# addtt/ladder-vae-pytorch

Hardware: AMD Instinct MI355X
Metric: training images/sec (ELBO step: fwd+bwd+Adamax) (higher is better)
Workload: dtype f32; 1 GPU; CIFAR10-shaped 15-layer LVAE (BASELINE configs[2]): 32x32x3, zdims 32x15, 4 blocks/layer, 64 filters, gated+skip, DMoL-10, dropout 0.2, free bits 1.0; batch_per_gpu=256, global_batch=256, parallelism=dp1, hip_graph=True

## Files before the change

### include/lvae_hip.h

```cpp
#ifndef LVAE_HIP_H
#define LVAE_HIP_H

#include <stddef.h>
#include <stdint.h>

#ifdef __cplusplus
extern "C" {
#endif

#define LVAE_ABI_VERSION 17

#define LVAE_EINVAL (-1)
#define LVAE_EALIGN (-2)
#define LVAE_EWORKSPACE (-3)

enum { LVAE_STATS_BN_FWD = 0, LVAE_STATS_BN_BWD = 1 };
enum { LVAE_PREC_F32 = 0, LVAE_PREC_BF16 = 1 };
enum { LVAE_DT_F32 = 0, LVAE_DT_BF16 = 1 };
enum {
  LVAE_FORM_AUTO = 0,
  LVAE_FORM_F32_MFMA = 1,
  LVAE_FORM_SIX_PRODUCT = 2,
  LVAE_FORM_SIX_PRODUCT_DIRECT = 3
};
// ... 87 lines not shown
  const float* coef;
  const float* dh;
  const float* x;
  const float* add;
  float* dgamma;
  float* dbeta;
  float* out;
  int32_t dh_bf16;
  int32_t reserved_;
  const float* drop;
} lvae_bn_apply;
size_t lvae_conv1x1_gate_bwd_wgrad_workspace(const lvae_conv_desc* d);
int lvae_conv1x1_gate_bwd_wgrad_f32(const lvae_conv_desc* d, const float* dout, const float* ab, const float* y, int32_t act,
                                    float* dw, int64_t dw_sk, int64_t dw_sn, float* db, void* workspace, size_t workspace_bytes,
                                    const lvae_bn_apply* ap, void* stream);

enum { LVAE_RB_PRO_AFFINE = 0, LVAE_RB_PRO_BN_APPLY = 1, LVAE_RB_PRO_GATE_BWD = 2 };
enum { LVAE_RB_EPI_PLAIN = 0, LVAE_RB_EPI_GATE = 1 };
typedef struct lvae_rb_ext {
  int32_t prologue, epilogue;
  const float* gate_w;
  int64_t gate_w_sk, gate_w_sn;
  void* gate_ws;
  int64_t gate_ws_bytes;
  int32_t gate_ws_ready;
  const float* gate_bias;
  int32_t act;
  const float* res;
  float* ab;
  float* out;
// ... 165 lines not shown
```

### ladder-vae-pytorch_amd/_C.py

```python
import ctypes as C
import os

import torch

_HERE = os.path.dirname(os.path.abspath(__file__))
LIB_PATH = os.path.join(_HERE, 'liblvae_hip.so')

ACT = {None: 0, 'none': 0, 'elu': 1, 'relu': 2, 'leakyrelu': 3, 'selu': 4}
GATHER_CONV, GATHER_TRANSPOSED = 0, 1
PREC_F32, PREC_BF16 = 0, 1
DT_F32, DT_BF16 = 0, 1
VARIANT_DIRECT, VARIANT_POS, VARIANT_WINO_F32, VARIANT_WINO_SIX, VARIANT_BF16_DIRECT, VARIANT_SIX_DIRECT = 0, 2, 3, 4, 5, 6
WGRAD_VARIANT_GENERIC, WGRAD_VARIANT_IMG, WGRAD_VARIANT_BF16, WGRAD_VARIANT_WINO, WGRAD_VARIANT_DIRECT_1X1, WGRAD_VARIANT_TILE, WGRAD_VARIANT_THIN = range(7)
FORM_AUTO, FORM_F32_MFMA, FORM_SIX_PRODUCT, FORM_SIX_PRODUCT_DIRECT = 0, 1, 2, 3


class LvaeHipError(RuntimeError):
    pass


class ConvDesc(C.Structure):
    _fields_ = [
        ('x', C.c_void_p), ('x2', C.c_void_p), ('C1', C.c_int32), ('C2', C.c_int32),
        ('w', C.c_void_p), ('w_stap', C.c_int64), ('w_sk', C.c_int64), ('w_sn', C.c_int64),
# ... 47 lines not shown
    'lvae_conv2d_bf16': (C.c_int, [C.POINTER(ConvDesc), _P]),
    'lvae_conv1x1_dgrad_cat_f32': (C.c_int, [C.POINTER(ConvDesc), _P, _I, _P]),
    'lvae_conv2d_stats_rows': (_I, [C.POINTER(ConvDesc)]),
    'lvae_conv2d_variant': (_I, [C.POINTER(ConvDesc)]),
    'lvae_resblock_bf16_storage': (_I, [C.POINTER(ConvDesc)]),
    'lvae_conv2d_folds_bn_finalize': (_I, [C.POINTER(ConvDesc)]),
    'lvae_conv2d_stats_buffer_rows': (_I, [C.POINTER(ConvDesc)]),
    'lvae_conv2d_prepare_entry_bytes': (_Z, []),
    'lvae_conv2d_prepare_entry': (C.c_int, [C.POINTER(ConvDesc), _P]),
    'lvae_conv2d_prepare_weights': (C.c_int, [_P, _I, _I, _P]),
    'lvae_conv1x1_gate_f32': (C.c_int, [C.POINTER(ConvDesc), _P, _I, _P, _P]),
    'lvae_conv1x1_gate_stats_rows': (_I, [C.POINTER(ConvDesc)]),
    'lvae_conv1x1_gate_bwd_f32': (C.c_int, [C.POINTER(ConvDesc), _P, _P, _I, _P, _P]),
    'lvae_conv1x1_gate_bwd_wgrad_workspace': (_Z, [C.POINTER(ConvDesc)]),
    'lvae_conv1x1_gate_bwd_wgrad_f32': (C.c_int, [C.POINTER(ConvDesc), _P, _P, _P, _I, _P, _L, _L, _P, _P, _Z, C.POINTER(BnApply), _P]),
    'lvae_resblock_gate_workspace': (_Z, [C.POINTER(ConvDesc)]),
    'lvae_resblock_gate_prepare_entry': (C.c_int, [C.POINTER(ConvDesc), _P]),
    'lvae_resblock_conv_rows': (_I, [C.POINTER(ConvDesc)]),
    'lvae_resblock_conv_gate_rows': (_I, [C.POINTER(ConvDesc)]),
    'lvae_resblock_conv_workspace': (_Z, [C.POINTER(ConvDesc)]),
    'lvae_resblock_conv_prepare_entry': (C.c_int, [C.POINTER(ConvDesc), _P]),
    'lvae_resblock_conv_f32': (C.c_int, [C.POINTER(ConvDesc), C.POINTER(RbExt), _P]),
    'lvae_conv2d_wgrad_workspace': (_Z, [C.POINTER(ConvDesc)]),
    'lvae_conv2d_wgrad_f32': (C.c_int, [C.POINTER(ConvDesc), _P, _P, _P, _P, _Z, _P]),
    'lvae_conv2d_wgrad_bf16': (C.c_int, [C.POINTER(ConvDesc), _P, _P, _P, _P, _Z, _P]),
    'lvae_conv2d_wgrad_variant': (_I, [C.POINTER(ConvDesc)]),
    'lvae_conv2d_wgrad_apply_ok': (_I, [C.POINTER(ConvDesc)]),
    'lvae_conv2d_wgrad_apply_f32': (C.c_int, [C.POINTER(ConvDesc), C.POINTER(BnApply), _P, _P, _P, _Z, _P]),
    'lvae_conv2d_wgrad_grouped_workspace': (_Z, [C.POINTER(ConvDesc), _I]),
    'lvae_conv2d_wgrad_grouped_f32': (C.c_int, [C.POINTER(ConvDesc), _P, _P, _P, _I, _P, _Z, _P]),
# ... 98 lines not shown
```

### ladder-vae-pytorch_amd/csrc/conv1x1_gate_bwd_fused.hip

```cpp
#include "bf16_frag.h"
#include "lvae_common.h"

namespace lvae {

void wgrad_reduce_launch(const float* slab_w, const float* slab_b, int ksplit, int ntaps, int Cin, int Cout, int64_t stap, int64_t sk,
                         int64_t sn, float* dw, float* db, hipStream_t s);

struct GbfArgs {
  const float* dout;
  const float* ab;
  const float* y;
  const float* w;
  int64_t w_sn;
  const float* drop;
  float* dx;
  float* slab_w;
  float* slab_b;
  int M, ohw, ntiles, act;
  int in_bf16, dx_bf16;
  lvae_bn_apply ap;
};

constexpr int GB_LDA = 132;
constexpr int GB_LDY = 68;

__global__ __launch_bounds__(512) void conv1x1_gate_bwd_fused_kernel(GbfArgs a) {
  kernarg_warmup<(sizeof(GbfArgs) < 1024 ? sizeof(GbfArgs) : 1024)>();
  extern __shared__ __attribute__((aligned(16))) float smem[];
  float* Bs = smem;
  float* As = Bs + 64 * GB_LDA;
  float* Ys = As + 64 * GB_LDA;
  const int t = threadIdx.x, lane = t & 63, wave = t >> 6;
  const bool wg_role = wave >= 4;
  const int wm = (wave & 3) >> 1, wn = wave & 1, li = lane & 31, lh = lane >> 5;
  const f32x4 zero4 = {0.f, 0.f, 0.f, 0.f};
// ... 106 lines not shown
    float* red = As;
    *reinterpret_cast<f32x4*>(red + r0 * 128 + c4) = bs_lo;
    *reinterpret_cast<f32x4*>(red + r0 * 128 + 64 + c4) = bs_hi;
    __syncthreads();
    if (t < 128) {
      float v = 0.f;
#pragma unroll
      for (int g = 0; g < 32; ++g) v += red[g * 128 + t];
      a.slab_b[(size_t)blockIdx.x * 128 + t] = v;
    }
  }
}

constexpr int GBB_LDA = 136;
constexpr int GBB_LDY = 72;
constexpr size_t gbb_lds(int split) {
  return (size_t)split * (64 * GBB_LDA + 64 * GBB_LDY) * 2 + (size_t)64 * GB_LDY * 4 + 6 * 64 * 4 + (split == 3 ? (size_t)8 * 2 * 3 * 64 * 16 : 0);
}

template <int SPLIT, bool S16 = false, bool AP = false, bool ELU = false>
__global__ __launch_bounds__(512) void conv1x1_gate_bwd_fused_bf16_kernel(GbfArgs a) {
  kernarg_warmup<sizeof(GbfArgs)>();
#ifdef LVAE_GBF_DBG
  constexpr int dbg = LVAE_GBF_DBG;
#else
  constexpr int dbg = 0;
#endif
  const int gact = ELU ? LVAE_ACT_ELU : a.act, apact = ELU ? LVAE_ACT_ELU : a.ap.act;
  static_assert(SPLIT == 1 || !S16, "bf16 storage exists for the bf16-operand form only");
  extern __shared__ __attribute__((aligned(16))) unsigned char smem_raw[];
  constexpr int A_PLANE = 64 * GBB_LDA, Y_PLANE = 64 * GBB_LDY;
  __bf16* As = reinterpret_cast<__bf16*>(smem_raw);
  __bf16* Ys = As + SPLIT * A_PLANE;
  float* Os = reinterpret_cast<float*>(Ys + SPLIT * Y_PLANE);
  float* Cf = Os + 64 * GB_LDY;
  const int t = threadIdx.x, lane = t & 63, wave = t >> 6;
  const bool wg_role = wave >= 4;
  const int wm = (wave & 3) >> 1, wn = wave & 1, li = lane & 31, lh = lane >> 5, G = lane >> 4, i16 = lane & 15;
  const f32x4 zero4 = {0.f, 0.f, 0.f, 0.f};

  if (AP) {
    const int q = t & 31, rg = t >> 5, rows = a.ap.rows;
    f32x4 acc = zero4;
    for (int r = rg; r < rows; r += 16 * 8) {
      f32x4 v[8];
#pragma unroll
      for (int u = 0; u < 8; ++u) {
        const int rr = r + 16 * u;
        v[u] = *reinterpret_cast<const f32x4*>(a.ap.parts + (size_t)(rr < rows ? rr : 0) * 128 + q * 4);
      }
// ... 60 lines not shown
  auto prefetch_row = [&](int tile, int u) {
    if (dbg & 1) {
      pg[u] = pa[u] = pb[u] = py[u] = zero4;
      if (AP) px[u] = pd[u] = zero4;
      return;
    }
    const int m = tile * 64 + r0 + 32 * u;
    const size_t mc = m < a.M ? (size_t)m : 0;
    if (AP) {
      pg[u] = load4_dt(a.ap.dh, mc * 64 + c4, ap_dh_bf);
      px[u] = *reinterpret_cast<const f32x4*>(a.ap.x + mc * 64 + c4);
      pd[u] = ap_add ? *reinterpret_cast<const f32x4*>(a.ap.add + mc * 64 + c4) : zero4;
    } else {
      pg[u] = *reinterpret_cast<const f32x4*>(a.dout + mc * 64 + c4);
    }
    pa[u] = load4_dt(a.ab, mc * 128 + c4, a.in_bf16 != 0);
    pb[u] = load4_dt(a.ab, mc * 128 + 64 + c4, a.in_bf16 != 0);
    py[u] = load4_dt(a.y, mc * 64 + c4, a.in_bf16 != 0);
  };
  auto prefetch = [&](int tile) {
    const int m0 = tile * 64;
    if (dbg & 1) {
      pg[0] = pg[1] = zero4;
#pragma unroll
      for (int u = 0; u < IT; ++u) pa[u] = pb[u] = py[u] = zero4;
#pragma unroll
      for (int u = 0; u < (AP ? 2 : 1); ++u) px[u] = pd[u] = zero4;
      qa = qb = qy = bf16x8{0, 0, 0, 0, 0, 0, 0, 0};
      return;
    }
    if (S16) {
      const int m = m0 + r8;
// ... 18 lines not shown
    for (int u = 0; u < IT; ++u) prefetch_row(tile, u);
  };

  f32x16 accw[2];
#pragma unroll
  for (int j = 0; j < 2; ++j)
#pragma unroll
    for (int r = 0; r < 16; ++r) accw[j][r] = 0.f;
  f32x4 bs_lo = zero4, bs_hi = zero4;
  f32x4 bs_lo8 = zero4, bs_hi8 = zero4;
  const int trow = 8 * (G >> 1) + (i16 >> 2), tch = 16 * (G & 1) + 4 * (i16 & 3);
  constexpr int NP = SPLIT == 1 ? 1 : 6;
  constexpr int PA[6] = {SPLIT - 1, 0, SPLIT > 1 ? 1 : 0, SPLIT > 1 ? 1 : 0, 0, 0};
  constexpr int PB[6] = {0, SPLIT - 1, SPLIT > 1 ? 1 : 0, 0, SPLIT > 1 ? 1 : 0, 0};

  int tile = blockIdx.x;
  if (tile < a.ntiles) prefetch(tile);
  for (; tile < a.ntiles; tile += gridDim.x) {
    const int m0 = tile * 64;
    if (S16) {
      f32x4 lo[2] = {zero4, zero4}, hi[2] = {zero4, zero4};
      bf16x8 yv = {0, 0, 0, 0, 0, 0, 0, 0};
      if (m0 + r8 < a.M) {
        if (AP) {
#pragma unroll
          for (int h = 0; h < 2; ++h) {
            pg[h] = ap_value(pg[h], px[h], pd[h], c8 + 4 * h);
            store_wt4(a.ap.out + (size_t)(m0 + r8) * 64 + c8 + 4 * h, pg[h]);
          }
        }
#pragma unroll
        for (int h = 0; h < 2; ++h)
#pragma unroll
          for (int j = 0; j < 4; ++j) {
// ... 9 lines not shown
      bs_hi += hi[0];
      bs_hi8 += hi[1];
      *reinterpret_cast<bf16x8*>(As + r8 * GBB_LDA + c8) = to_bf16x8(lo[0], lo[1]);
      *reinterpret_cast<bf16x8*>(As + r8 * GBB_LDA + 64 + c8) = to_bf16x8(hi[0], hi[1]);
      *reinterpret_cast<bf16x8*>(Ys + r8 * GBB_LDY + c8) = yv;
    } else
#pragma unroll
    for (int u = 0; u < IT; ++u) {
      const int r = r0 + 32 * u;
      f32x4 lo = zero4, hi = zero4, yv = zero4;
      if (m0 + r < a.M) {
        if (AP) {
          pg[u] = ap_value(pg[u], px[u], pd[u], c4);
          if (!(dbg & 4)) store_wt4(a.ap.out + (size_t)(m0 + r) * 64 + c4, pg[u]);
        }
        if (dbg & 8) {
          lo = pg[u] + pa[u];
          hi = pg[u] + pb[u];
        } else
#pragma unroll
        for (int j = 0; j < 4; ++j) {
          const float sg = sigmoidf_(pb[u][j]);
          lo[j] = pg[u][j] * sg * act_grad(pa[u][j], gact);
          hi[j] = pg[u][j] * act_fwd(pa[u][j], gact) * sg * (1.f - sg);
        }
        yv = py[u];
      }
      bs_lo += lo;
      bs_hi += hi;
      if (tile + (int)gridDim.x < a.ntiles) prefetch_row(tile + gridDim.x, u);
      bf16x4 pl[SPLIT], ph[SPLIT], pyv[SPLIT];
      split4<SPLIT>(lo, pl);
      split4<SPLIT>(hi, ph);
      split4<SPLIT>(yv, pyv);
#pragma unroll
      for (int q = 0; q < SPLIT; ++q) {
        *reinterpret_cast<bf16x4*>(As + q * A_PLANE + r * GBB_LDA + c4) = pl[q];
        *reinterpret_cast<bf16x4*>(As + q * A_PLANE + r * GBB_LDA + 64 + c4) = ph[q];
        *reinterpret_cast<bf16x4*>(Ys + q * Y_PLANE + r * GBB_LDY + c4) = pyv[q];
      }
    }
    if (S16 && tile + (int)gridDim.x < a.ntiles) prefetch(tile + gridDim.x);
    lds_barrier();

    if (!wg_role) {
      f32x16 accx;
#pragma unroll
      for (int r = 0; r < 16; ++r) accx[r] = 0.f;
#pragma unroll
      for (int s = 0; s < 8; ++s) {
        bf16x8 af[SPLIT];
#pragma unroll
        for (int q = 0; q < SPLIT; ++q)
          af[q] = *reinterpret_cast<const bf16x8*>(As + q * A_PLANE + (wm * 32 + li) * GBB_LDA + 16 * s + 8 * lh);
// ... 101 lines not shown
  return (int)(ntiles < 256 ? ntiles : 256);
}

size_t conv1x1_gate_bwd_fused_workspace(const lvae_conv_desc* d) {
  static const bool off = tune("LVAE_DISABLE_GATE_FUSED", 0) != 0;
  if (off || d == nullptr) return 0;
  if (d->KH != 1 || d->KW != 1 || d->stride != 1 || d->pad != 0 || d->OH != d->H || d->OW != d->W) return 0;
  if (d->C1 != 128 || d->C2 != 0 || d->Cout != 64 || d->w_sk != 1 || d->w_sn % 4 != 0 || d->in_scale != nullptr) return 0;
  const int64_t M = (int64_t)d->N * d->H * d->W;
  static const int64_t min_m = tune("LVAE_GATE_FUSED_MIN_M", 256 * 64);
  if (M < min_m || M >= ((int64_t)1 << 31)) return 0;
  return (size_t)gbf_nwg(M) * (64 * 128 + 128) * sizeof(float);
}

int conv1x1_gate_bwd_fused(const lvae_conv_desc* d, const float* dout, const float* ab, const float* y, int act, float* dw,
                           int64_t dw_sk, int64_t dw_sn, float* db, void* workspace, const lvae_bn_apply* ap, hipStream_t s) {
  if (!al16f(dout) || !al16f(ab) || !al16f(y) || !al16f(d->w) || !al16f(d->y) || !al16f(d->out_scale) || !al16f(workspace)) return -1000;
  GbfArgs a;
  a.ap = lvae_bn_apply{};
  if (ap != nullptr && ap->parts != nullptr) {
    if (!al16f(ap->parts) || !al16f(ap->coef) || !al16f(ap->dh) || !al16f(ap->x) || !al16f(ap->add) || !al16f(ap->out)) return -1000;
    a.ap = *ap;
  }
  a.dout = dout;
  a.ab = ab;
  a.y = y;
  a.w = d->w;
  a.w_sn = d->w_sn;
  a.drop = d->out_scale;
  a.dx = d->y;
  a.M = d->N * d->H * d->W;
  a.ohw = d->H * d->W;
  a.ntiles = (a.M + 63) / 64;
  a.act = act;
  a.in_bf16 = d->x_dtype == LVAE_DT_BF16;
  a.dx_bf16 = d->y_dtype == LVAE_DT_BF16;
  if ((a.in_bf16 || a.dx_bf16) && d->precision != LVAE_PREC_BF16) return -1000;
  const int nwg = gbf_nwg(a.M);
  a.slab_w = static_cast<float*>(workspace);
  a.slab_b = db ? a.slab_w + (size_t)nwg * 64 * 128 : nullptr;
  constexpr size_t lds = (size_t)(2 * 64 * GB_LDA + 64 * GB_LDY) * sizeof(float);
  static std::atomic<bool> attr_set{false};
  if (!attr_set) {
    hipError_t e = hipFuncSetAttribute(reinterpret_cast<const void*>(conv1x1_gate_bwd_fused_kernel),
                                       hipFuncAttributeMaxDynamicSharedMemorySize, (int)lds);
    if (e != hipSuccess) {
      set_error("conv1x1_gate_bwd_fused: hipFuncSetAttribute failed: %s", hipGetErrorString(e));
      return (int)e;
    }
    attr_set = true;
  }
  const bool f32_mfma = d->form == LVAE_FORM_F32_MFMA;
  const bool with_ap = a.ap.parts != nullptr;
  if (with_ap && (f32_mfma && d->precision != LVAE_PREC_BF16)) {
    set_error("conv1x1_gate_bwd_fused: the deferred BatchNorm-backward apply exists in the bf16-matrix-pipe kernels only (not with LVAE_FORM_F32_MFMA)");
    return LVAE_EINVAL;
  }
  const bool elu = act == LVAE_ACT_ELU && (!with_ap || a.ap.act == LVAE_ACT_ELU);
#define GBF_LAUNCH(SP, S16_, AP_, LDS_)                                                                                                   \
  do {                                                                                                                                    \
    if (elu) hipLaunchKernelGGL((conv1x1_gate_bwd_fused_bf16_kernel<SP, S16_, AP_, true>), dim3(nwg), dim3(512), LDS_, s, a);            \
    else hipLaunchKernelGGL((conv1x1_gate_bwd_fused_bf16_kernel<SP, S16_, AP_, false>), dim3(nwg), dim3(512), LDS_, s, a);               \
  } while (0)
  if (d->precision == LVAE_PREC_BF16) {
    if (with_ap) {
      if (a.in_bf16 && a.dx_bf16) GBF_LAUNCH(1, true, true, gbb_lds(1));
      else GBF_LAUNCH(1, false, true, gbb_lds(1));
    } else if (a.in_bf16 && a.dx_bf16) GBF_LAUNCH(1, true, false, gbb_lds(1));
    else GBF_LAUNCH(1, false, false, gbb_lds(1));
  } else if (!f32_mfma) {
    static std::atomic<bool> attr3_set{false};
    if (!attr3_set) {
      hipError_t e = hipSuccess;
      const void* ks[4] = {(const void*)conv1x1_gate_bwd_fused_bf16_kernel<3, false, false, false>, (const void*)conv1x1_gate_bwd_fused_bf16_kernel<3, false, false, true>,
                           (const void*)conv1x1_gate_bwd_fused_bf16_kernel<3, false, true, false>, (const void*)conv1x1_gate_bwd_fused_bf16_kernel<3, false, true, true>};
      for (int i = 0; i < 4 && e == hipSuccess; ++i) e = hipFuncSetAttribute(ks[i], hipFuncAttributeMaxDynamicSharedMemorySize, (int)gbb_lds(3));
      if (e != hipSuccess) {
        set_error("conv1x1_gate_bwd_fused: hipFuncSetAttribute failed: %s", hipGetErrorString(e));
        return (int)e;
      }
      attr3_set = true;
    }
    if (with_ap) GBF_LAUNCH(3, false, true, gbb_lds(3));
    else GBF_LAUNCH(3, false, false, gbb_lds(3));
#undef GBF_LAUNCH
  } else {
    hipLaunchKernelGGL(conv1x1_gate_bwd_fused_kernel, dim3(nwg), dim3(512), lds, s, a);
  }
  LVAE_LAUNCH_CHECK("conv1x1_gate_bwd_fused");
  wgrad_reduce_launch(a.slab_w, a.slab_b, nwg, 1, 64, 128, 0, dw_sk, dw_sn, dw, db, s);
  LVAE_LAUNCH_CHECK("conv1x1_gate_bwd_fused_reduce");
  return 0;
}

}

using namespace lvae;

extern "C" size_t lvae_conv1x1_gate_bwd_wgrad_workspace(const lvae_conv_desc* d) { return conv1x1_gate_bwd_fused_workspace(d); }

extern "C" int lvae_conv1x1_gate_bwd_wgrad_f32(const lvae_conv_desc* d, const float* dout, const float* ab, const float* y, int32_t act,
                                               float* dw, int64_t dw_sk, int64_t dw_sn, float* db, void* workspace,
                                               size_t workspace_bytes, const lvae_bn_apply* ap, void* stream) {
  const bool with_ap = ap != nullptr && ap->parts != nullptr;
  LVAE_REQUIRE(d && (dout || with_ap) && ab && y && d->y && dw && workspace, LVAE_EINVAL, "lvae_conv1x1_gate_bwd_wgrad_f32: null pointer");
  if (with_ap)
    LVAE_REQUIRE(ap->rows > 0 && ap->M == (int64_t)d->N * d->H * d->W && ap->coef && ap->dh && ap->x && ap->out, LVAE_EINVAL,
                 "lvae_conv1x1_gate_bwd_wgrad_f32: deferred apply needs parts / rows, M = N*H*W, the coefficient block, dh, x and out");
  const size_t need = conv1x1_gate_bwd_fused_workspace(d);
  LVAE_REQUIRE(need > 0, LVAE_EINVAL,
               "lvae_conv1x1_gate_bwd_wgrad_f32: unsupported shape (needs the gate of a 64-channel block: 1x1, 128 -> 64 dgrad view, at "
               "least 16384 pixels); use lvae_conv1x1_gate_bwd_f32 + lvae_conv2d_wgrad_f32");
  LVAE_REQUIRE(workspace_bytes >= need, LVAE_EWORKSPACE, "lvae_conv1x1_gate_bwd_wgrad_f32: workspace %zu < %zu", workspace_bytes, need);
  const int rc = conv1x1_gate_bwd_fused(d, dout, ab, y, act, dw, dw_sk, dw_sn, db, workspace, ap, (hipStream_t)stream);
  LVAE_REQUIRE(rc != -1000, LVAE_EALIGN, "lvae_conv1x1_gate_bwd_wgrad_f32: buffers must be 16-byte aligned");
  return rc;
}
```

### ladder-vae-pytorch_amd/kernels.py

```python
import ctypes as C
import weakref

import torch

from . import _C
from ._C import ACT, BnFold, ConvDesc, RbExt, GATHER_CONV, GATHER_TRANSPOSED, PREC_BF16, PREC_F32, call, ptr, ptr_dt, stream_ptr

_ws_cache = {}

precision = PREC_F32


form = _C.FORM_AUTO


class use_form:
    def __init__(self, f):
        self.f = f

    def __enter__(self):
        global form
        self.prev, form = form, self.f

    def __exit__(self, *exc):
# ... 319 lines not shown
    dx = torch.empty((N, H, W, g.Cin), dtype=torch.bfloat16 if out_bf16 else torch.float32, device=dout.device)
    d = _desc(g, weight, ab, None, N, H, W, H, W, g.Cin, g.s_co, g.s_ci, GATHER_TRANSPOSED, out_scale=out_scale, y=dx)
    need = _C.load().lvae_conv1x1_gate_bwd_wgrad_workspace(C.byref(d))
    if not need or (apply is not None and form == _C.FORM_F32_MFMA and precision != PREC_BF16):
        return None
    ws = workspace(need, dout.device)
    ap = None
    if apply is not None:
        ap = _C.BnApply(ptr(apply.parts), apply.parts.shape[0], ACT[apply.act], N * H * W, ptr(apply.coef0), ptr_dt(apply.dh), ptr(apply.x),
                        ptr(apply.add), ptr(apply.dgamma), ptr(apply.dbeta), ptr(apply.out), int(apply.dh.dtype == torch.bfloat16), 0)
    call('lvae_conv1x1_gate_bwd_wgrad_f32', C.byref(d), ptr(dout), ptr_dt(ab), ptr_dt(y), ACT[act], ptr(dweight), g.s_ci, g.s_co, ptr(dbias),
         ws.data_ptr(), ws.numel(), C.byref(ap) if ap is not None else None, stream_ptr())
    return dx


def _rb_desc(x_like, weight, g, dgrad, y=None, bias=None, in_scale=None, in_shift=None, in_act=None, out_scale=None):
    N, H, W, _ = x_like.shape
    if dgrad:
        d = _desc(g, weight, x_like, None, N, H, W, H, W, g.Cin, g.s_co, g.s_ci, GATHER_TRANSPOSED, out_scale=out_scale, y=y)
    else:
        d = _desc(g, weight, x_like, None, N, H, W, H, W, g.Cout, g.s_ci, g.s_co, GATHER_CONV, bias, in_scale, in_shift, in_act, out_scale, None, y)
    need = _C.load().lvae_resblock_conv_workspace(C.byref(d))
    if need:
        prepared.attach(d, weight, x_like.device, need, 'lvae_resblock_conv_prepare_entry')
    return d, need


def _rb_gate_ws(e, gate_w, gate_g, device, bwd):
    gd = ConvDesc()
    gd.w, gd.precision = ptr(gate_w), precision
# ... 85 lines not shown


def rb_gate_rows(x, weight, g):
    if _ddi is not None or x.dtype != torch.float32 or x.dim() != 4 or g.transposed or g.KH != 3 or g.stride != 1 or g.pad != 1:
        return 0
    N, H, W, _ = x.shape
    d = _desc(g, weight, x, None, N, H, W, H, W, g.Cout, g.s_ci, g.s_co, GATHER_CONV)
    rows = int(_C.load().lvae_resblock_conv_rows(C.byref(d)))
    if rows > 0:
        return rows
    _conv_ws(d, weight, x.device)
    return int(_C.load().lvae_resblock_conv_gate_rows(C.byref(d)))


def rb_conv_gate(x, weight, g, bias, in_act, out_scale, gate_w, gate_g, gate_bias, res, act, in_bn=None, coef=None, stats_pivot=None,
                 prefetch=None):
    N, H, W, _ = x.shape
    dev = x.device
    y = torch.empty((N, H, W, g.Cout), dtype=torch.float32, device=dev)
    ab = torch.empty((N, H, W, gate_g.Cout), dtype=torch.float32, device=dev)
    out = torch.empty((N, H, W, gate_g.Cout // 2), dtype=torch.float32, device=dev)
    d, need = _rb_desc(x, weight, g, False, y, bias, None, None, in_act, out_scale)
    can_fold = True
    if not need:
        _conv_ws(d, weight, dev)
        can_fold = bool(_C.load().lvae_conv2d_folds_bn_finalize(C.byref(d)))
    keep = None
    if in_bn is not None:
        coef, keep = _rb_in_bn(d, in_bn, x, can_fold)
    else:
        d.in_scale, d.in_shift = ptr(coef[0]), ptr(coef[1])
    e = RbExt()
    e.prologue, e.epilogue = _C.RB_PRO_AFFINE, _C.RB_EPI_GATE
    _rb_gate_ws(e, gate_w, gate_g, dev, False)
    e.gate_bias, e.act = ptr(gate_bias), ACT[act]
    e.res, e.ab, e.out = ptr(res), ptr(ab), ptr(out)
    parts = None
# ... 538 lines not shown
```

### ladder-vae-pytorch_amd/ops.py

```python
import os

import torch
from torch.autograd import Function

from . import kernels as K

_const_cache = {}


def _ones_zeros(C, device):
    key = (C, device)
    if key not in _const_cache:
        _const_cache[key] = (torch.ones(C, device=device), torch.zeros(C, device=device))
    return _const_cache[key]


def grad_buf(p):
    if not p.requires_grad:
        return None
    if p.grad is None:
        p.grad = torch.zeros_like(p)
    return p.grad


# ... 97 lines not shown
            if both is not None:
                dx, dx2 = both
            else:
                if ctx.needs_input_grad[0]:
                    dx = K.conv2d_dgrad(dy, w, g, hw, ci_range=(0, C1))
                if ctx.needs_input_grad[1]:
                    dx2 = K.conv2d_dgrad(dy, w, g, hw, ci_range=(C1, g.Cin))
        return dx, dx2, None, None, None, None


def conv(x, mod, x2=None, out_act=None):
    return ConvFn.apply(x, x2, mod, out_act, mod.weight, mod.bias)


_GATE_STATS = os.environ.get('LVAE_NO_GATE_STATS') is None


import weakref as _weakref

_rb_chain = {'fwd': None, 'bwd': None}


def _rb_link(direction, blk, first_ranges):
    blk.__dict__['_rb_first_' + direction] = first_ranges
    prev = _rb_chain[direction]
    prev = prev() if prev is not None else None
    if prev is not None and prev is not blk:
        prev.__dict__['_rb_next_' + direction] = _weakref.ref(blk)
    _rb_chain[direction] = _weakref.ref(blk)

# ... 24 lines not shown
        dev = x.device
        C = x.shape[3]
        st = []
        h = x
        parts, pivot_in = blk.__dict__.pop('_in_parts', None) or (None, None)
        full = (training and blk.gate is not None and blk.bn1 is not None and blk.bn2 is not None and blk.gate.bias is not None and
                blk.conv1.bias is not None and blk.conv2.bias is not None and blk.bn1.running_mean is not None and
                blk.bn2.running_mean is not None and x.dtype == torch.float32)
        rb_fwd, rb_bwd = K.rb_policy(x, blk.conv1.weight, blk.conv1.geom()) if full else (False, False)
        if rb_fwd:
            return ResBlockFn._forward_fused(ctx, x, blk, m1, m2, parts, pivot_in, rb_bwd)
        s16 = (not rb_bwd and blk.gate is not None and blk.bn1 is not None and blk.bn2 is not None and blk.gate.bias is not None and
               (training or not torch.is_grad_enabled()) and K.resblock_bf16_storage(x, blk.conv1.weight, blk.conv1.geom()))
        fuse_gate = bool(full and not s16 and K._RB_GATE_LARGE and K.rb_rows(x, blk.conv2.weight, blk.conv2.geom()) == 0 and
                         K.rb_gate_rows(x, blk.conv2.weight, blk.conv2.geom()) > 0)
        fused_out = None
        for i, (bn, cv, m) in enumerate(((blk.bn1, blk.conv1, m1), (blk.bn2, blk.conv2, m2))):
            nxt = blk.bn2 if i == 0 else None
            want_stats = training and nxt is not None and nxt.running_mean is not None
            if i == 1 and fuse_gate:
                in_bn = coef = None
                if parts is not None:
                    in_bn = (parts, bn.running_mean, bn)
                else:
                    coef = K.bn_stats(h, bn.weight, bn.bias, bn.running_mean, bn.running_var, bn.eps, bn.momentum)
                pivot = st[0][3].detach() if (st[0][3] is not None and _GATE_STATS) else None
                gate = blk.gate
                y, ab_f, out_f, oparts_f, (sc, sh, mean, rstd) = K.rb_conv_gate(
                    h, cv.weight, cv.geom(), cv.bias, act, m, gate.weight, gate.geom(), gate.bias, x, act, in_bn=in_bn, coef=coef, stats_pivot=pivot)
                fused_out = (ab_f, out_f, oparts_f, pivot)
                st.append((h, sc, sh, mean, rstd))
                h = y
                continue
            if bn is not None and training and parts is not None:
                y, parts_out, (sc, sh, mean, rstd) = K.conv2d(
                    h, cv.weight, cv.geom(), bias=cv.bias, in_act=act, out_scale=m, in_bn=(parts, pivot_in if i == 0 else bn.running_mean, bn),
                    stats_pivot=nxt.running_mean if want_stats else None, out_bf16=s16)
            else:
                if bn is not None:
                    if training:
                        sc, sh, mean, rstd = K.bn_stats(h, bn.weight, bn.bias, bn.running_mean, bn.running_var, bn.eps, bn.momentum)
                    else:
                        sc, sh = K.bn_eval_coeffs(bn.weight, bn.bias, bn.running_mean, bn.running_var, bn.eps)
                        mean = rstd = None
# ... 14 lines not shown
        blk.__dict__['_out_parts'] = None
        if fused_out is not None:
            ab, out, oparts, pivot = fused_out
            if oparts is not None:
                blk.__dict__['_out_parts'] = (oparts, pivot)
        elif blk.gate is not None:
            if training and blk.bn1 is not None and blk.bn1.running_mean is not None and _GATE_STATS:
                pivot = st[0][3].detach() if st[0][3] is not None else blk.bn1.running_mean.clone()
                ab, out, oparts = K.conv1x1_gate(y2, blk.gate.weight, blk.gate.geom(), blk.gate.bias, x, act, stats_pivot=pivot)
                if oparts is not None:
                    blk.__dict__['_out_parts'] = (oparts, pivot)
            else:
                ab, out = K.conv1x1_gate(y2, blk.gate.weight, blk.gate.geom(), blk.gate.bias, x, act)
        else:
            out = K.add(y2, x)
        ctx.blk, ctx.training, ctx.s16 = blk, training, s16
        (x0, sc1, sh1, mean1, rstd1), (y1, sc2, sh2, mean2, rstd2) = st
        ctx.rb_bwd = bool(rb_bwd and ab is not None and K.bn_coef_block(sc1, sh1, mean1, rstd1) and K.bn_coef_block(sc2, sh2, mean2, rstd2))
        ctx.defer_to = blk.__dict__.pop('_in_src', None)
        acc = 'f32-dh' if ctx.rb_bwd else None
        if (not ctx.rb_bwd and _DEFER_LARGE and training and blk.gate is not None and blk.gate.bias is not None and blk.gate.weight.requires_grad and
                ab is not None and K.gate_bwd_fused_ok(x, blk.gate.weight, blk.gate.geom())):
            acc = 'any-dh'
        blk.__dict__['_accepts_deferred'] = acc
        ctx.save_for_backward(x0, y1, y2, ab, sc1, sh1, mean1, rstd1, sc2, sh2, mean2, rstd2, m1, m2)
        return out

    @staticmethod
    def _forward_fused(ctx, x, blk, m1, m2, parts, pivot_in, rb_bwd):
        act = blk.act
        bn1, bn2, cv1, cv2, gate = blk.bn1, blk.bn2, blk.conv1, blk.conv2, blk.gate
        in_bn = coef1 = None
        if parts is not None and parts.has_pivot:
            in_bn = (parts, pivot_in, bn1)
        elif parts is not None:
            N, H, W, _ = x.shape
            coef1 = K.bn_finalize_parts(parts.rows_view(), N * H * W, pivot_in, bn1.weight, bn1.bias, bn1.running_mean, bn1.running_var,
                                        bn1.eps, bn1.momentum)
        else:
            coef1 = K.bn_stats(x, bn1.weight, bn1.bias, bn1.running_mean, bn1.running_var, bn1.eps, bn1.momentum)
        _rb_link('fwd', blk, K.rb_weight_ranges(x, cv1.weight, cv1.geom(), False))
        nxt = K.rb_weight_ranges(x, cv2.weight, cv2.geom(), False, gate=(gate.weight, gate.geom()))
        y1, parts2, coef1 = K.rb_conv(x, cv1.weight, cv1.geom(), cv1.bias, act, m1, in_bn=in_bn, coef=coef1, stats_pivot=bn2.running_mean,
                                      prefetch=nxt)
        blk.__dict__['_out_parts'] = None
        pivot = coef1[2].detach() if _GATE_STATS else None
        y2, ab, out, oparts, coef2 = K.rb_conv_gate(y1, cv2.weight, cv2.geom(), cv2.bias, act, m2, gate.weight, gate.geom(), gate.bias, x, act,
                                                    in_bn=(parts2, bn2.running_mean, bn2), stats_pivot=pivot,
                                                    prefetch=_rb_next_ranges('fwd', blk))
        if oparts is not None:
            blk.__dict__['_out_parts'] = (oparts, pivot)
        ctx.blk, ctx.training, ctx.s16 = blk, True, False
        ctx.rb_bwd = bool(rb_bwd and K.bn_coef_block(*coef1) and K.bn_coef_block(*coef2))
        ctx.defer_to = blk.__dict__.pop('_in_src', None)
        blk.__dict__['_accepts_deferred'] = 'f32-dh' if ctx.rb_bwd else None
        ctx.save_for_backward(x, y1, y2, ab, coef1[0], coef1[1], coef1[2], coef1[3], coef2[0], coef2[1], coef2[2], coef2[3], m1, m2)
        return out

    @staticmethod
    def backward(ctx, dout):
        blk = ctx.blk
        act = blk.act
        x, y1, y2, ab, sc1, sh1, mean1, rstd1, sc2, sh2, mean2, rstd2, m1, m2 = ctx.saved_tensors
        dout = _c(dout)
        hw = (x.shape[1], x.shape[2])
        s16 = ctx.s16
        if ctx.rb_bwd:
# ... 3 lines not shown
            dab, dy2, dh2, parts2 = K.rb_gate_dgrad(dout, ab, gw, gate.geom(), act, m2, w2, blk.conv2.geom(), bn_bwd=(y1, sc2, act),
                                                    prefetch=K.rb_weight_ranges(dout, w1, blk.conv1.geom(), True), apply=_take_pending(blk, dout))
            if gw.requires_grad:
                wgrad(y2, dab, gw, gate.geom(), grad_buf(gw), grad_buf(gate.bias))
            wgrad(y1, dy2, w2, blk.conv2.geom(), grad_buf(w2), grad_buf(blk.conv2.bias), in_scale=sc2, in_shift=sh2, in_act=act)
            dy1, dh1, parts1 = K.rb_apply_dgrad(parts2, dh2, y1, sc2, act, grad_buf(bn2.weight), grad_buf(bn2.bias), m1, w1, blk.conv1.geom(),
                                                bn_bwd=(x, sc1, act), prefetch=_rb_next_ranges('bwd', blk))
            wgrad(x, dy1, w1, blk.conv1.geom(), grad_buf(w1), grad_buf(blk.conv1.bias), in_scale=sc1, in_shift=sh1, in_act=act)
            dx = ResBlockFn._final_apply(ctx, parts1, dh1, x, sc1, sh1, mean1, rstd1, act, bn1, dout)
            return (dx, None, None, None, None) + (None,) * (len(ctx.needs_input_grad) - 5)
        pend = _take_pending(blk, dout)
        if blk.gate is not None:
            gw = blk.gate.weight
            dy2 = None
            if gw.requires_grad and blk.gate.bias is not None:
                dy2 = K.conv1x1_gate_bwd_wgrad(dout, ab, y2, gw, blk.gate.geom(), act, grad_buf(gw), grad_buf(blk.gate.bias), out_scale=m2,
                                               out_bf16=s16, apply=pend)
                if dy2 is not None:
                    pend = None
            if pend is not None:
                pend = ResBlockFn._run_pending(pend)
            if dy2 is None:
                if s16:
                    raise K._C.LvaeHipError("bf16-stored residual block: the fused gate backward did not take this shape")
                dab, dy2 = K.conv1x1_gate_bwd(dout, ab, gw, blk.gate.geom(), act, out_scale=m2)
                wgrad(y2, dab, gw, blk.gate.geom(), grad_buf(gw), grad_buf(blk.gate.bias))
        else:
            if pend is not None:
                pend = ResBlockFn._run_pending(pend)
            dy2 = K.scale_rows_add(dout, m2, None) if m2 is not None else dout
        w2 = blk.conv2.weight
        wgrad(y1, dy2, w2, blk.conv2.geom(), grad_buf(w2), grad_buf(blk.conv2.bias), in_scale=sc2, in_shift=sh2, in_act=act)
# ... 382 lines not shown
```

Measured before the change: 8955 images/s.

## Recompute gate pre-activations in fused gate backward instead of storing ab

Adds a recompute form of the fused 1x1 gate backward kernel. Instead of reading the stored 128-channel gate pre-activation tensor ab, it rebuilds ab from y via an extra six-product bf16-split MFMA GEMM with the prepared gate weights plus bias. The forward pass then skips allocating and writing ab for these blocks. This trades extra matrix work and a larger LDS footprint per block for less HBM write and read traffic and lower activation memory.

```diff
diff --git a/include/lvae_hip.h b/include/lvae_hip.h
--- a/include/lvae_hip.h
+++ b/include/lvae_hip.h
@@ -125,6 +125,11 @@
 int lvae_conv1x1_gate_bwd_wgrad_f32(const lvae_conv_desc* d, const float* dout, const float* ab, const float* y, int32_t act,
                                     float* dw, int64_t dw_sk, int64_t dw_sn, float* db, void* workspace, size_t workspace_bytes,
                                     const lvae_bn_apply* ap, void* stream);
+size_t lvae_conv1x1_gate_bwd_recompute_workspace(const lvae_conv_desc* d);
+int lvae_conv1x1_gate_bwd_recompute_f32(const lvae_conv_desc* d, const float* dout, const float* y, void* gate_ws, size_t gate_ws_bytes,
+                                        int32_t gate_ws_ready, const float* gate_bias, int32_t act, float* dw, int64_t dw_sk,
+                                        int64_t dw_sn, float* db, void* workspace, size_t workspace_bytes, const lvae_bn_apply* ap,
+                                        void* stream);
 
 enum { LVAE_RB_PRO_AFFINE = 0, LVAE_RB_PRO_BN_APPLY = 1, LVAE_RB_PRO_GATE_BWD = 2 };
 enum { LVAE_RB_EPI_PLAIN = 0, LVAE_RB_EPI_GATE = 1 };
diff --git a/ladder-vae-pytorch_amd/_C.py b/ladder-vae-pytorch_amd/_C.py
--- a/ladder-vae-pytorch_amd/_C.py
+++ b/ladder-vae-pytorch_amd/_C.py
@@ -85,6 +85,9 @@
     'lvae_conv1x1_gate_bwd_f32': (C.c_int, [C.POINTER(ConvDesc), _P, _P, _I, _P, _P]),
     'lvae_conv1x1_gate_bwd_wgrad_workspace': (_Z, [C.POINTER(ConvDesc)]),
     'lvae_conv1x1_gate_bwd_wgrad_f32': (C.c_int, [C.POINTER(ConvDesc), _P, _P, _P, _I, _P, _L, _L, _P, _P, _Z, C.POINTER(BnApply), _P]),
+    'lvae_conv1x1_gate_bwd_recompute_workspace': (_Z, [C.POINTER(ConvDesc)]),
+    'lvae_conv1x1_gate_bwd_recompute_f32': (C.c_int, [C.POINTER(ConvDesc), _P, _P, _P, _Z, _I, _P, _I, _P, _L, _L, _P, _P, _Z,
+                                                      C.POINTER(BnApply), _P]),
     'lvae_resblock_gate_workspace': (_Z, [C.POINTER(ConvDesc)]),
     'lvae_resblock_gate_prepare_entry': (C.c_int, [C.POINTER(ConvDesc), _P]),
     'lvae_resblock_conv_rows': (_I, [C.POINTER(ConvDesc)]),
diff --git a/ladder-vae-pytorch_amd/csrc/conv1x1_gate_bwd_fused.hip b/ladder-vae-pytorch_amd/csrc/conv1x1_gate_bwd_fused.hip
--- a/ladder-vae-pytorch_amd/csrc/conv1x1_gate_bwd_fused.hip
+++ b/ladder-vae-pytorch_amd/csrc/conv1x1_gate_bwd_fused.hip
@@ -19,6 +19,8 @@
   int M, ohw, ntiles, act;
   int in_bf16, dx_bf16;
   lvae_bn_apply ap;
+  const __bf16* gws;
+  const float* gbias;
 };
 
 constexpr int GB_LDA = 132;
@@ -155,12 +157,16 @@
 
 constexpr int GBB_LDA = 136;
 constexpr int GBB_LDY = 72;
-constexpr size_t gbb_lds(int split) {
-  return (size_t)split * (64 * GBB_LDA + 64 * GBB_LDY) * 2 + (size_t)64 * GB_LDY * 4 + 6 * 64 * 4 + (split == 3 ? (size_t)8 * 2 * 3 * 64 * 16 : 0);
-}
-
-template <int SPLIT, bool S16 = false, bool AP = false, bool ELU = false>
+constexpr int GBB_LDQ = 128;
+constexpr size_t gbb_os_bytes(bool rc) { return rc ? (size_t)64 * GBB_LDQ * 4 : (size_t)64 * GB_LDY * 4; }
+constexpr size_t gbb_lds(int split, bool rc = false) {
+  return (size_t)split * (64 * GBB_LDA + 64 * GBB_LDY) * 2 + gbb_os_bytes(rc) + 6 * 64 * 4 + (split == 3 ? (size_t)8 * 2 * 3 * 64 * 16 : 0);
+}
+static_assert(gbb_lds(3, true) <= 160 * 1024, "recompute form exceeds the LDS of a CU");
+
+template <int SPLIT, bool S16 = false, bool AP = false, bool ELU = false, bool RC = false>
 __global__ __launch_bounds__(512) void conv1x1_gate_bwd_fused_bf16_kernel(GbfArgs a) {
+  static_assert(!RC || (SPLIT == 3 && !S16), "the recompute form mirrors the fp32 (six-product) gate epilogue");
   kernarg_warmup<sizeof(GbfArgs)>();
 #ifdef LVAE_GBF_DBG
   constexpr int dbg = LVAE_GBF_DBG;
@@ -174,7 +180,7 @@
   __bf16* As = reinterpret_cast<__bf16*>(smem_raw);
   __bf16* Ys = As + SPLIT * A_PLANE;
   float* Os = reinterpret_cast<float*>(Ys + SPLIT * Y_PLANE);
-  float* Cf = Os + 64 * GB_LDY;
+  float* Cf = Os + gbb_os_bytes(RC) / 4;
   const int t = threadIdx.x, lane = t & 63, wave = t >> 6;
   const bool wg_role = wave >= 4;
   const int wm = (wave & 3) >> 1, wn = wave & 1, li = lane & 31, lh = lane >> 5, G = lane >> 4, i16 = lane & 15;
@@ -265,8 +271,10 @@
     } else {
       pg[u] = *reinterpret_cast<const f32x4*>(a.dout + mc * 64 + c4);
     }
-    pa[u] = load4_dt(a.ab, mc * 128 + c4, a.in_bf16 != 0);
-    pb[u] = load4_dt(a.ab, mc * 128 + 64 + c4, a.in_bf16 != 0);
+    if (!RC) {
+      pa[u] = load4_dt(a.ab, mc * 128 + c4, a.in_bf16 != 0);
+      pb[u] = load4_dt(a.ab, mc * 128 + 64 + c4, a.in_bf16 != 0);
+    }
     py[u] = load4_dt(a.y, mc * 64 + c4, a.in_bf16 != 0);
   };
   auto prefetch = [&](int tile) {
@@ -315,10 +323,52 @@
   constexpr int PA[6] = {SPLIT - 1, 0, SPLIT > 1 ? 1 : 0, SPLIT > 1 ? 1 : 0, 0, 0};
   constexpr int PB[6] = {0, SPLIT - 1, SPLIT > 1 ? 1 : 0, 0, SPLIT > 1 ? 1 : 0, 0};
 
+  float* Qs = Os;
+  f32x4 gba = zero4, gbb = zero4;
+  if (RC && a.gbias) {
+    gba = *reinterpret_cast<const f32x4*>(a.gbias + c4);
+    gbb = *reinterpret_cast<const f32x4*>(a.gbias + 64 + c4);
+  }
+
   int tile = blockIdx.x;
   if (tile < a.ntiles) prefetch(tile);
   for (; tile < a.ntiles; tile += gridDim.x) {
     const int m0 = tile * 64;
+    if (RC) {
+      const int gct = 2 * (wave >> 2) + wn;
+      bf16x8 gq[4][3];
+      const __bf16* gp = a.gws + (size_t)gct * 3 * 512 + lane * 8;
+#pragma unroll
+      for (int s4 = 0; s4 < 4; ++s4)
+#pragma unroll
+        for (int q = 0; q < 3; ++q) gq[s4][q] = *reinterpret_cast<const bf16x8*>(gp + (size_t)(s4 * 12 + q) * 512);
+#pragma unroll
+      for (int u = 0; u < IT; ++u) {
+        const int r = r0 + 32 * u;
+        bf16x4 pyv[3];
+        split4<3>(m0 + r < a.M ? py[u] : zero4, pyv);
+#pragma unroll
+        for (int q = 0; q < 3; ++q) *reinterpret_cast<bf16x4*>(Ys + q * Y_PLANE + r * GBB_LDY + c4) = pyv[q];
+      }
+      lds_barrier();
+      f32x16 acq;
+#pragma unroll
+      for (int r = 0; r < 16; ++r) acq[r] = 0.f;
+#pragma unroll
+      for (int s4 = 0; s4 < 4; ++s4) {
+        bf16x8 af[3];
+#pragma unroll
+        for (int q = 0; q < 3; ++q) af[q] = *reinterpret_cast<const bf16x8*>(Ys + q * Y_PLANE + (wm * 32 + li) * GBB_LDY + 16 * s4 + 8 * lh);
+#pragma unroll
+        for (int k = 0; k < 6; ++k) {
+          if (dbg & 2) acq[k] += (float)af[PA[k]][0] * (float)gq[s4][PB[k]][1];
+          else acq = __builtin_amdgcn_mfma_f32_32x32x16_bf16(af[PA[k]], gq[s4][PB[k]], acq, 0, 0, 0);
+        }
+      }
+#pragma unroll
+      for (int r = 0; r < 16; ++r) Qs[(wm * 32 + (r & 3) + 8 * (r >> 2) + 4 * lh) * GBB_LDQ + 32 * gct + li] = acq[r];
+      lds_barrier();
+    }
     if (S16) {
       f32x4 lo[2] = {zero4, zero4}, hi[2] = {zero4, zero4};
       bf16x8 yv = {0, 0, 0, 0, 0, 0, 0, 0};
@@ -358,6 +408,10 @@
           pg[u] = ap_value(pg[u], px[u], pd[u], c4);
           if (!(dbg & 4)) store_wt4(a.ap.out + (size_t)(m0 + r) * 64 + c4, pg[u]);
         }
+        if (RC) {
+          pa[u] = *reinterpret_cast<const f32x4*>(Qs + r * GBB_LDQ + c4) + gba;
+          pb[u] = *reinterpret_cast<const f32x4*>(Qs + r * GBB_LDQ + 64 + c4) + gbb;
+        }
         if (dbg & 8) {
           lo = pg[u] + pa[u];
           hi = pg[u] + pb[u];
@@ -376,12 +430,12 @@
       bf16x4 pl[SPLIT], ph[SPLIT], pyv[SPLIT];
       split4<SPLIT>(lo, pl);
       split4<SPLIT>(hi, ph);
-      split4<SPLIT>(yv, pyv);
+      if (!RC) split4<SPLIT>(yv, pyv);
 #pragma unroll
       for (int q = 0; q < SPLIT; ++q) {
         *reinterpret_cast<bf16x4*>(As + q * A_PLANE + r * GBB_LDA + c4) = pl[q];
         *reinterpret_cast<bf16x4*>(As + q * A_PLANE + r * GBB_LDA + 64 + c4) = ph[q];
-        *reinterpret_cast<bf16x4*>(Ys + q * Y_PLANE + r * GBB_LDY + c4) = pyv[q];
+        if (!RC) *reinterpret_cast<bf16x4*>(Ys + q * Y_PLANE + r * GBB_LDY + c4) = pyv[q];
       }
     }
     if (S16 && tile + (int)gridDim.x < a.ntiles) prefetch(tile + gridDim.x);
@@ -513,8 +567,11 @@
 }
 
 int conv1x1_gate_bwd_fused(const lvae_conv_desc* d, const float* dout, const float* ab, const float* y, int act, float* dw,
-                           int64_t dw_sk, int64_t dw_sn, float* db, void* workspace, const lvae_bn_apply* ap, hipStream_t s) {
+                           int64_t dw_sk, int64_t dw_sn, float* db, void* workspace, const lvae_bn_apply* ap, hipStream_t s,
+                           const __bf16* gws = nullptr, const float* gbias = nullptr) {
   if (!al16f(dout) || !al16f(ab) || !al16f(y) || !al16f(d->w) || !al16f(d->y) || !al16f(d->out_scale) || !al16f(workspace)) return -1000;
+  if (!al16f(gws) || !al16f(gbias)) return -1000;
+  const bool rc = ab == nullptr;
   GbfArgs a;
   a.ap = lvae_bn_apply{};
   if (ap != nullptr && ap->parts != nullptr) {
@@ -523,6 +580,8 @@
   }
   a.dout = dout;
   a.ab = ab;
+  a.gws = gws;
+  a.gbias = gbias;
   a.y = y;
   a.w = d->w;
   a.w_sn = d->w_sn;
@@ -535,6 +594,10 @@
   a.in_bf16 = d->x_dtype == LVAE_DT_BF16;
   a.dx_bf16 = d->y_dtype == LVAE_DT_BF16;
   if ((a.in_bf16 || a.dx_bf16) && d->precision != LVAE_PREC_BF16) return -1000;
+  if (rc && (a.in_bf16 || a.dx_bf16 || d->precision != LVAE_PREC_F32 || d->form == LVAE_FORM_F32_MFMA || gws == nullptr)) {
+    set_error("conv1x1_gate_bwd_fused: the recompute form exists for fp32 storage in the six-product form only");
+    return LVAE_EINVAL;
+  }
   const int nwg = gbf_nwg(a.M);
   a.slab_w = static_cast<float*>(workspace);
   a.slab_b = db ? a.slab_w + (size_t)nwg * 64 * 128 : nullptr;
@@ -556,10 +619,10 @@
     return LVAE_EINVAL;
   }
   const bool elu = act == LVAE_ACT_ELU && (!with_ap || a.ap.act == LVAE_ACT_ELU);
-#define GBF_LAUNCH(SP, S16_, AP_, LDS_)                                                                                                   \
+#define GBF_LAUNCH(SP, S16_, AP_, LDS_, ...)                                                                                              \
   do {                                                                                                                                    \
-    if (elu) hipLaunchKernelGGL((conv1x1_gate_bwd_fused_bf16_kernel<SP, S16_, AP_, true>), dim3(nwg), dim3(512), LDS_, s, a);            \
-    else hipLaunchKernelGGL((conv1x1_gate_bwd_fused_bf16_kernel<SP, S16_, AP_, false>), dim3(nwg), dim3(512), LDS_, s, a);               \
+    if (elu) hipLaunchKernelGGL((conv1x1_gate_bwd_fused_bf16_kernel<SP, S16_, AP_, true, ##__VA_ARGS__>), dim3(nwg), dim3(512), LDS_, s, a); \
+    else hipLaunchKernelGGL((conv1x1_gate_bwd_fused_bf16_kernel<SP, S16_, AP_, false, ##__VA_ARGS__>), dim3(nwg), dim3(512), LDS_, s, a);    \
   } while (0)
   if (d->precision == LVAE_PREC_BF16) {
     if (with_ap) {
@@ -567,6 +630,23 @@
       else GBF_LAUNCH(1, false, true, gbb_lds(1));
     } else if (a.in_bf16 && a.dx_bf16) GBF_LAUNCH(1, true, false, gbb_lds(1));
     else GBF_LAUNCH(1, false, false, gbb_lds(1));
+  } else if (rc) {
+    static std::atomic<bool> attr_rc_set{false};
+    if (!attr_rc_set) {
+      hipError_t e = hipSuccess;
+      const void* ks[4] = {(const void*)conv1x1_gate_bwd_fused_bf16_kernel<3, false, false, false, true>,
+                           (const void*)conv1x1_gate_bwd_fused_bf16_kernel<3, false, false, true, true>,
+                           (const void*)conv1x1_gate_bwd_fused_bf16_kernel<3, false, true, false, true>,
+                           (const void*)conv1x1_gate_bwd_fused_bf16_kernel<3, false, true, true, true>};
+      for (int i = 0; i < 4 && e == hipSuccess; ++i) e = hipFuncSetAttribute(ks[i], hipFuncAttributeMaxDynamicSharedMemorySize, (int)gbb_lds(3, true));
+      if (e != hipSuccess) {
+        set_error("conv1x1_gate_bwd_fused: hipFuncSetAttribute failed: %s", hipGetErrorString(e));
+        return (int)e;
+      }
+      attr_rc_set = true;
+    }
+    if (with_ap) GBF_LAUNCH(3, false, true, gbb_lds(3, true), true);
+    else GBF_LAUNCH(3, false, false, gbb_lds(3, true), true);
   } else if (!f32_mfma) {
     static std::atomic<bool> attr3_set{false};
     if (!attr3_set) {
@@ -591,6 +671,15 @@
   LVAE_LAUNCH_CHECK("conv1x1_gate_bwd_fused_reduce");
   return 0;
 }
+
+size_t conv1x1_gate_bwd_recompute_workspace(const lvae_conv_desc* d) {
+  if (d == nullptr || d->precision != LVAE_PREC_F32 || d->form == LVAE_FORM_F32_MFMA || d->x_dtype != LVAE_DT_F32 || d->y_dtype != LVAE_DT_F32)
+    return 0;
+  return conv1x1_gate_bwd_fused_workspace(d);
+}
+
+size_t resblock_gate_ws_bytes(const lvae_conv_desc* d, int planes);
+int resblock_gate_prepare_single(const lvae_conv_desc* d, int planes, hipStream_t s);
 
 }
 
@@ -615,3 +704,41 @@
   LVAE_REQUIRE(rc != -1000, LVAE_EALIGN, "lvae_conv1x1_gate_bwd_wgrad_f32: buffers must be 16-byte aligned");
   return rc;
 }
+
+extern "C" size_t lvae_conv1x1_gate_bwd_recompute_workspace(const lvae_conv_desc* d) { return conv1x1_gate_bwd_recompute_workspace(d); }
+
+extern "C" int lvae_conv1x1_gate_bwd_recompute_f32(const lvae_conv_desc* d, const float* dout, const float* y, void* gate_ws,
+                                                   size_t gate_ws_bytes, int32_t gate_ws_ready, const float* gate_bias, int32_t act,
+                                                   float* dw, int64_t dw_sk, int64_t dw_sn, float* db, void* workspace,
+                                                   size_t workspace_bytes, const lvae_bn_apply* ap, void* stream) {
+  const bool with_ap = ap != nullptr && ap->parts != nullptr;
+  LVAE_REQUIRE(d && (dout || with_ap) && y && d->y && d->w && gate_ws && dw && workspace, LVAE_EINVAL,
+               "lvae_conv1x1_gate_bwd_recompute_f32: null pointer");
+  if (with_ap)
+    LVAE_REQUIRE(ap->rows > 0 && ap->M == (int64_t)d->N * d->H * d->W && ap->coef && ap->dh && ap->x && ap->out, LVAE_EINVAL,
+                 "lvae_conv1x1_gate_bwd_recompute_f32: deferred apply needs parts / rows, M = N*H*W, the coefficient block, dh, x and out");
+  const size_t need = conv1x1_gate_bwd_recompute_workspace(d);
+  LVAE_REQUIRE(need > 0, LVAE_EINVAL,
+               "lvae_conv1x1_gate_bwd_recompute_f32: unsupported descriptor (needs lvae_conv1x1_gate_bwd_wgrad_workspace's shapes, fp32 "
+               "storage, precision LVAE_PREC_F32, not LVAE_FORM_F32_MFMA); use lvae_conv1x1_gate_bwd_wgrad_f32 with the stored ab");
+  LVAE_REQUIRE(workspace_bytes >= need, LVAE_EWORKSPACE, "lvae_conv1x1_gate_bwd_recompute_f32: workspace %zu < %zu", workspace_bytes, need);
+  lvae_conv_desc g = lvae_conv_desc{};
+  g.w = d->w;
+  g.w_sk = d->w_sn;
+  g.w_sn = d->w_sk;
+  g.C1 = 64;
+  g.Cout = 128;
+  g.precision = LVAE_PREC_F32;
+  g.workspace = gate_ws;
+  g.workspace_bytes = gate_ws_bytes;
+  LVAE_REQUIRE(gate_ws_bytes >= resblock_gate_ws_bytes(&g, 3), LVAE_EWORKSPACE, "lvae_conv1x1_gate_bwd_recompute_f32: gate_ws %zu < %zu",
+               gate_ws_bytes, resblock_gate_ws_bytes(&g, 3));
+  if (!gate_ws_ready) {
+    const int rc = resblock_gate_prepare_single(&g, 3, (hipStream_t)stream);
+    if (rc) return rc;
+  }
+  const int rc = conv1x1_gate_bwd_fused(d, dout, nullptr, y, act, dw, dw_sk, dw_sn, db, workspace, ap, (hipStream_t)stream,
+                                        static_cast<const __bf16*>(gate_ws), gate_bias);
+  LVAE_REQUIRE(rc != -1000, LVAE_EALIGN, "lvae_conv1x1_gate_bwd_recompute_f32: buffers must be 16-byte aligned");
+  return rc;
+}
diff --git a/ladder-vae-pytorch_amd/kernels.py b/ladder-vae-pytorch_amd/kernels.py
--- a/ladder-vae-pytorch_amd/kernels.py
+++ b/ladder-vae-pytorch_amd/kernels.py
@@ -357,6 +357,45 @@
     return dx
 
 
+def _gate_recompute_desc(y, weight, g, out_scale=None, dx=None):
+    N, H, W, _ = y.shape
+    d = _desc(g, weight, y, None, N, H, W, H, W, g.Cin, g.s_co, g.s_ci, GATHER_TRANSPOSED, out_scale=out_scale, y=dx)
+    d.C1 = g.Cout
+    return d
+
+
+def gate_bwd_recompute_ok(x_like, weight, g):
+    N, H, W, Cn = x_like.shape
+    if not (g.KH == 1 and g.KW == 1 and g.stride == 1 and g.pad == 0 and not g.transposed and g.Cout == 2 * Cn and g.s_co == 1):
+        return False
+    if x_like.dtype != torch.float32:
+        return False
+    return bool(_C.load().lvae_conv1x1_gate_bwd_recompute_workspace(C.byref(_gate_recompute_desc(x_like, weight, g))))
+
+
+def conv1x1_gate_bwd_recompute(dout, y, weight, g, gate_bias, act, dweight, dbias, out_scale=None, apply=None):
+    _chk_nhwc(dout, 'dout')
+    if tuple(dweight.stride()) != tuple(weight.stride()):
+        raise _C.LvaeHipError("conv1x1_gate_bwd_recompute: dweight must have the weight's strides")
+    N, H, W, Cn = dout.shape
+    dx = torch.empty((N, H, W, g.Cin), dtype=torch.float32, device=dout.device)
+    d = _gate_recompute_desc(y, weight, g, out_scale, dx)
+    need = _C.load().lvae_conv1x1_gate_bwd_recompute_workspace(C.byref(d))
+    if not need:
+        raise _C.LvaeHipError("conv1x1_gate_bwd_recompute: the recompute form does not take this gate convolution")
+    ws = workspace(need, dout.device)
+    e = RbExt()
+    _rb_gate_ws(e, weight, g, dout.device, False)
+    ap = None
+    if apply is not None:
+        ap = _C.BnApply(ptr(apply.parts), apply.parts.shape[0], ACT[apply.act], N * H * W, ptr(apply.coef0), ptr_dt(apply.dh), ptr(apply.x),
+                        ptr(apply.add), ptr(apply.dgamma), ptr(apply.dbeta), ptr(apply.out), int(apply.dh.dtype == torch.bfloat16), 0)
+    call('lvae_conv1x1_gate_bwd_recompute_f32', C.byref(d), ptr(dout), ptr(y), e.gate_ws, e.gate_ws_bytes, e.gate_ws_ready, ptr(gate_bias),
+         ACT[act], ptr(dweight), g.s_ci, g.s_co, ptr(dbias), ws.data_ptr(), ws.numel(), C.byref(ap) if ap is not None else None, stream_ptr())
+    del e
+    return dx
+
+
 def _rb_desc(x_like, weight, g, dgrad, y=None, bias=None, in_scale=None, in_shift=None, in_act=None, out_scale=None):
     N, H, W, _ = x_like.shape
     if dgrad:
@@ -472,13 +511,15 @@
 
 
 def rb_conv_gate(x, weight, g, bias, in_act, out_scale, gate_w, gate_g, gate_bias, res, act, in_bn=None, coef=None, stats_pivot=None,
-                 prefetch=None):
+                 prefetch=None, want_ab=True):
     N, H, W, _ = x.shape
     dev = x.device
     y = torch.empty((N, H, W, g.Cout), dtype=torch.float32, device=dev)
-    ab = torch.empty((N, H, W, gate_g.Cout), dtype=torch.float32, device=dev)
+    ab = torch.empty((N, H, W, gate_g.Cout), dtype=torch.float32, device=dev) if want_ab else None
     out = torch.empty((N, H, W, gate_g.Cout // 2), dtype=torch.float32, device=dev)
     d, need = _rb_desc(x, weight, g, False, y, bias, None, None, in_act, out_scale)
+    if need and not want_ab:
+        raise _C.LvaeHipError("rb_conv_gate: the whole-image kernels always store ab")
     can_fold = True
     if not need:
         _conv_ws(d, weight, dev)
diff --git a/ladder-vae-pytorch_amd/ops.py b/ladder-vae-pytorch_amd/ops.py
--- a/ladder-vae-pytorch_amd/ops.py
+++ b/ladder-vae-pytorch_amd/ops.py
@@ -135,6 +135,7 @@
 
 
 _GATE_STATS = os.environ.get('LVAE_NO_GATE_STATS') is None
+_GATE_RECOMPUTE = True
 
 
 import weakref as _weakref
@@ -189,6 +190,8 @@
                (training or not torch.is_grad_enabled()) and K.resblock_bf16_storage(x, blk.conv1.weight, blk.conv1.geom()))
         fuse_gate = bool(full and not s16 and K._RB_GATE_LARGE and K.rb_rows(x, blk.conv2.weight, blk.conv2.geom()) == 0 and
                          K.rb_gate_rows(x, blk.conv2.weight, blk.conv2.geom()) > 0)
+        recompute = bool(fuse_gate and _GATE_RECOMPUTE and not rb_bwd and blk.gate.weight.requires_grad and
+                         K.gate_bwd_recompute_ok(x, blk.gate.weight, blk.gate.geom()))
         fused_out = None
         for i, (bn, cv, m) in enumerate(((blk.bn1, blk.conv1, m1), (blk.bn2, blk.conv2, m2))):
             nxt = blk.bn2 if i == 0 else None
@@ -202,7 +205,8 @@
                 pivot = st[0][3].detach() if (st[0][3] is not None and _GATE_STATS) else None
                 gate = blk.gate
                 y, ab_f, out_f, oparts_f, (sc, sh, mean, rstd) = K.rb_conv_gate(
-                    h, cv.weight, cv.geom(), cv.bias, act, m, gate.weight, gate.geom(), gate.bias, x, act, in_bn=in_bn, coef=coef, stats_pivot=pivot)
+                    h, cv.weight, cv.geom(), cv.bias, act, m, gate.weight, gate.geom(), gate.bias, x, act, in_bn=in_bn, coef=coef, stats_pivot=pivot,
+                    want_ab=not recompute)
                 fused_out = (ab_f, out_f, oparts_f, pivot)
                 st.append((h, sc, sh, mean, rstd))
                 h = y
@@ -247,13 +251,13 @@
                 ab, out = K.conv1x1_gate(y2, blk.gate.weight, blk.gate.geom(), blk.gate.bias, x, act)
         else:
             out = K.add(y2, x)
-        ctx.blk, ctx.training, ctx.s16 = blk, training, s16
+        ctx.blk, ctx.training, ctx.s16, ctx.gate_recompute = blk, training, s16, recompute
         (x0, sc1, sh1, mean1, rstd1), (y1, sc2, sh2, mean2, rstd2) = st
         ctx.rb_bwd = bool(rb_bwd and ab is not None and K.bn_coef_block(sc1, sh1, mean1, rstd1) and K.bn_coef_block(sc2, sh2, mean2, rstd2))
         ctx.defer_to = blk.__dict__.pop('_in_src', None)
         acc = 'f32-dh' if ctx.rb_bwd else None
         if (not ctx.rb_bwd and _DEFER_LARGE and training and blk.gate is not None and blk.gate.bias is not None and blk.gate.weight.requires_grad and
-                ab is not None and K.gate_bwd_fused_ok(x, blk.gate.weight, blk.gate.geom())):
+                (ab is not None or recompute) and K.gate_bwd_fused_ok(x, blk.gate.weight, blk.gate.geom())):
             acc = 'any-dh'
         blk.__dict__['_accepts_deferred'] = acc
         ctx.save_for_backward(x0, y1, y2, ab, sc1, sh1, mean1, rstd1, sc2, sh2, mean2, rstd2, m1, m2)
@@ -283,7 +287,7 @@
                                                     prefetch=_rb_next_ranges('fwd', blk))
         if oparts is not None:
             blk.__dict__['_out_parts'] = (oparts, pivot)
-        ctx.blk, ctx.training, ctx.s16 = blk, True, False
+        ctx.blk, ctx.training, ctx.s16, ctx.gate_recompute = blk, True, False, False
         ctx.rb_bwd = bool(rb_bwd and K.bn_coef_block(*coef1) and K.bn_coef_block(*coef2))
         ctx.defer_to = blk.__dict__.pop('_in_src', None)
         blk.__dict__['_accepts_deferred'] = 'f32-dh' if ctx.rb_bwd else None
@@ -317,8 +321,12 @@
             gw = blk.gate.weight
             dy2 = None
             if gw.requires_grad and blk.gate.bias is not None:
-                dy2 = K.conv1x1_gate_bwd_wgrad(dout, ab, y2, gw, blk.gate.geom(), act, grad_buf(gw), grad_buf(blk.gate.bias), out_scale=m2,
-                                               out_bf16=s16, apply=pend)
+                if ctx.gate_recompute:
+                    dy2 = K.conv1x1_gate_bwd_recompute(dout, y2, gw, blk.gate.geom(), blk.gate.bias, act, grad_buf(gw), grad_buf(blk.gate.bias),
+                                                       out_scale=m2, apply=pend)
+                else:
+                    dy2 = K.conv1x1_gate_bwd_wgrad(dout, ab, y2, gw, blk.gate.geom(), act, grad_buf(gw), grad_buf(blk.gate.bias), out_scale=m2,
+                                                   out_bf16=s16, apply=pend)
                 if dy2 is not None:
                     pend = None
             if pend is not None:
```

Measured after the change: 8992 images/s, median of 6. About the same (+0.4%).
